# anibali/dsnt-pose2d

Hardware: AMD Instinct MI355X
Metric: images/sec (train step, 256x256, 16 joints) (higher is better)
Workload: dtype f32; 1 GPU; hg2 + DSNT + JS reg, 256x256 -> 64x64x16, batch 32 per GPU, RMSprop lr 2.5e-4, train step fwd+loss+bwd+optim; global_batch=32, parallelism=dp1, launches_fwd=212

## Files before the change

dsnt-pose2d_amd/csrc/api.cpp:

```cpp
#include "common.h"
#include "stage.h"
#include <string.h>

static thread_local char g_err[512] = "";

int dsnt_set_error(int code, const char* fmt, ...) {
    va_list ap;
    va_start(ap, fmt);
    vsnprintf(g_err, sizeof(g_err), fmt, ap);
    va_end(ap);
    return code;
}

int dsnt_device_id(void) {
    int d = 0;
    if (hipGetDevice(&d) != hipSuccess || d < 0) d = 0;
    return d < DSNT_MAX_DEVICES ? d : DSNT_MAX_DEVICES - 1;
}

int dsnt_device_cus(void) {
    static std::atomic<int> cus[DSNT_MAX_DEVICES];
    const int d = dsnt_device_id();
    int c = cus[d].load(std::memory_order_acquire);
    if (!c) {
        hipDeviceProp_t prop;
        int dev = 0;
        c = (hipGetDevice(&dev) == hipSuccess && hipGetDeviceProperties(&prop, dev) == hipSuccess && prop.multiProcessorCount > 0)
                ? prop.multiProcessorCount : 256;
        cus[d].store(c, std::memory_order_release);
    }
    return c;
}

extern "C" int dsnt_version(void) { return 121; }
extern "C" const char* dsnt_last_error(void) { return g_err; }

#include <vector>
#include <new>

struct dsnt_list {
    struct Entry {
        int kind;
        int lane, src, dst;
        mutable hipEvent_t ev;
        std::function<void(hipStream_t)> fn;
        int st_code = 0, gx = 0, gy = 0, nt = 0;
        std::vector<unsigned char> params;
        int fused = 0;
        unsigned* st_sync = nullptr;
// ... 202 lines not shown
```

dsnt-pose2d_amd/csrc/head.hip:

```cpp
#include "common.h"
#include "flipmerge.h"
#include <math.h>

#define HB 256

template <int VEC, bool CACHED, typename SRC = const float*>
struct Row {
    float v[16];
    SRC src;
    int hw;
    __device__ __forceinline__ void load(SRC row, int n) {
        src = row; hw = n;
        if (CACHED) {
            const int tid = threadIdx.x;
            if (VEC == 4) {
#pragma unroll
                for (int k = 0; k < 4; ++k) {
                    const int i = (k * HB + tid) * 4;
                    float4 t = make_float4(0.f, 0.f, 0.f, 0.f);
                    if (i < hw) t = row_load4(row, i);
                    v[4 * k] = t.x; v[4 * k + 1] = t.y; v[4 * k + 2] = t.z; v[4 * k + 3] = t.w;
                }
            } else {
#pragma unroll
// ... 612 lines not shown
        float x, y; g.xy(i, x, y);
        float v = ax * x + ay * y;
        if (kind >= 0 && gr != 0.f) v += gr * reg_grad(p, x, y, c, tx, ty, k, sigma, kind);
        return v;
    };
    float s[1] = {0.f};
    row.each([&](int i, float p) { s[0] = fmaf(p, dLdp(i, p), s[0]); });
    block_sum<1>(s, red);
    float* out = g_logits + r * hw;
    row.each([&](int i, float p) { out[i] = p * (dLdp(i, p) - s[0]); });
}

#define HEAD_SEP_MAX 512
#define LN2 0.69314718055994530942f

template <int VEC>
__global__ __launch_bounds__(HB) void head_loss_grad_kernel(const float* __restrict__ hm, const float* __restrict__ coords,
                                                            const float* __restrict__ target, const float* __restrict__ mask,
                                                            const float* __restrict__ denom_p, float* __restrict__ dist_out,
                                                            float* __restrict__ reg_out, float* __restrict__ g0, int h, int w,
                                                            float sigma, float k, int kind, float reg_coeff) {
    __shared__ float red[16];
    __shared__ __attribute__((aligned(16))) float exy[HEAD_SEP_MAX];
    __shared__ __attribute__((aligned(16))) float pos[HEAD_SEP_MAX];
    const size_t r = blockIdx.x;
    const int hw = h * w;
    const float tx = target[2 * r], ty = target[2 * r + 1];
    const float cx = coords[2 * r], cy = coords[2 * r + 1];
    const float mk = mask ? mask[r] : 1.f;
    const float den = denom_p[1];
    Row<VEC, true> row;
    row.load(hm + r * hw, hw);
    const Grid2 g(h, w);
    const float dxm = cx - tx, dym = cy - ty;
    const float d = sqrtf(dxm * dxm + dym * dym);
    const float wm = mk / den;
    const float f = wm / (2.f * d);
    const float ax = f * (2.f * dxm), ay = f * (2.f * dym);
    const float gr = kind >= 0 ? wm * reg_coeff : 0.f;
    float gv[16];
    float acc[2] = {0.f, 0.f};
    const bool tab = w + h <= HEAD_SEP_MAX;
    if (tab) {
        for (int i = threadIdx.x; i < w + h; i += HB)
            pos[i] = i < w ? (2.f * i - g.offx) / (float)w : (2.f * (i - w) - g.offy) / (float)h;
    }
    if (kind == 0 && tab) {
// ... 87 lines not shown
                    const float4 xv = *reinterpret_cast<const float4*>(pos + cc);
                    one(4 * kk, row.v[4 * kk], xv.x, y); one(4 * kk + 1, row.v[4 * kk + 1], xv.y, y);
                    one(4 * kk + 2, row.v[4 * kk + 2], xv.z, y); one(4 * kk + 3, row.v[4 * kk + 3], xv.w, y);
                }
            }
        } else {
            row.each_slot([&](int slot, int i, float p) {
                float x, y; g.xy(i, x, y);
                one(slot, p, x, y);
            });
        }
        float s1[1] = {acc[1]};
        block_sum<1>(s1, red);
        acc[0] = val; acc[1] = s1[0];
    }
    float* out = g0 + r * hw;
    if (VEC == 4) {
#pragma unroll
        for (int kk = 0; kk < 4; ++kk) {
            const int i = (kk * HB + threadIdx.x) * 4;
            if (i < hw)
                *reinterpret_cast<float4*>(out + i) = make_float4(row.v[4 * kk] * (gv[4 * kk] - acc[1]), row.v[4 * kk + 1] * (gv[4 * kk + 1] - acc[1]),
                                                                  row.v[4 * kk + 2] * (gv[4 * kk + 2] - acc[1]), row.v[4 * kk + 3] * (gv[4 * kk + 3] - acc[1]));
        }
    } else {
        row.each_slot([&](int slot, int i, float p) { out[i] = p * (gv[slot] - acc[1]); });
    }
    if (threadIdx.x == 0) {
        dist_out[r] = d;
        if (reg_out) reg_out[r] = acc[0];
    }
}

__global__ __launch_bounds__(HB) void mask_denom_kernel(const float* __restrict__ m, float* __restrict__ out2, long n) {
    __shared__ float red[16];
    float s[1] = {0.f};
    for (long i = threadIdx.x; i < n; i += HB) s[0] += m ? m[i] : 1.f;
    block_sum<1>(s, red);
    if (threadIdx.x == 0) { out2[0] = s[0]; out2[1] = fmaxf(s[0], 1.f); }
}

__global__ __launch_bounds__(HB) void head_loss_reduce_kernel(const float* __restrict__ dist, const float* __restrict__ reg,
                                                              const float* __restrict__ m, const float* __restrict__ denom2,
                                                              float reg_coeff, float* __restrict__ loss, float* __restrict__ e2,
                                                              long n) {
    __shared__ float red[16];
// ... 11 lines not shown
        loss[0] = reg ? a + reg_coeff * (s[1] / den) : a;
    }
}

__global__ void scale_by_scalar_kernel(float* __restrict__ x, const float* __restrict__ s, long n4, long n) {
    const float a = s[0];
    if (a == 1.f) return;
    const long t0 = (long)blockIdx.x * blockDim.x + threadIdx.x, step = (long)gridDim.x * blockDim.x;
    float4* x4 = reinterpret_cast<float4*>(x);
    for (long i = t0; i < n4; i += step) {
        float4 v = x4[i];
        v.x *= a; v.y *= a; v.z *= a; v.w *= a;
        x4[i] = v;
    }
    for (long i = 4 * n4 + t0; i < n; i += step) x[i] *= a;
}

#define ROW_DISPATCH(KERNEL, rows, hw, ptr_ok, ...)                                                   \
    do {                                                                                               \
        const bool vec_ = ((hw) % 4 == 0) && (ptr_ok);                                                 \
        const bool cached_ = (hw) <= 4096;                                                             \
        hipStream_t st_ = (hipStream_t)stream;                                                         \
        if (vec_ && cached_) DSNT_LAUNCH((KERNEL<4, true>), dim3(rows), dim3(HB), 0, st_, __VA_ARGS__);   \
        else if (cached_) DSNT_LAUNCH((KERNEL<1, true>), dim3(rows), dim3(HB), 0, st_, __VA_ARGS__);      \
        else DSNT_LAUNCH((KERNEL<1, false>), dim3(rows), dim3(HB), 0, st_, __VA_ARGS__);                  \
    } while (0)

static int check_rows(const char* who, int64_t rows, int h, int w) {
    DSNT_REQUIRE(rows > 0 && rows < (1LL << 31), DSNT_ERR_SHAPE, "%s: rows=%lld out of range", who, (long long)rows);
    DSNT_REQUIRE(h > 0 && w > 0 && (long)h * w < (1L << 24), DSNT_ERR_SHAPE, "%s: bad map size %dx%d", who, h, w);
// ... 301 lines not shown
    DSNT_REQUIRE(dist && denom2 && loss && e2 && rows > 0, DSNT_ERR_ARG, "dsnt_head_loss_reduce: bad argument");
    DSNT_LAUNCH(head_loss_reduce_kernel, dim3(1), dim3(HB), 0, (hipStream_t)stream, dist, reg_row, mask, denom2, reg_coeff,
                       loss, e2, (long)rows);
    DSNT_CHECK_LAUNCH("dsnt_head_loss_reduce");
}

extern "C" int dsnt_scale_by_scalar(float* x, const float* s, int64_t n, void* stream) {
    DSNT_REQUIRE(x && s && n > 0, DSNT_ERR_ARG, "dsnt_scale_by_scalar: null pointer or n <= 0");
    const long n4 = dsnt_aligned16(x) ? (long)(n / 4) : 0;
    long gsz = ((n4 ? n4 : (long)n) + 255) / 256;
    if (gsz > 4096) gsz = 4096;
    DSNT_LAUNCH(scale_by_scalar_kernel, dim3((unsigned)gsz), dim3(256), 0, (hipStream_t)stream, x, s, n4, (long)n);
    DSNT_CHECK_LAUNCH("dsnt_scale_by_scalar");
}

__global__ __launch_bounds__(256) void fc2_fwd_kernel(const float* __restrict__ hm, const float* __restrict__ w,
                                                      const float* __restrict__ b, float* __restrict__ out, int hw) {
    __shared__ float red[2][4];
    const float* row = hm + (size_t)blockIdx.x * hw;
    float a0 = 0.f, a1 = 0.f;
    for (int i = threadIdx.x; i < hw; i += 256) {
        const float v = row[i];
        a0 = fmaf(v, w[i], a0);
        a1 = fmaf(v, w[hw + i], a1);
    }
    for (int o = 32; o >= 1; o >>= 1) { a0 += __shfl_xor(a0, o); a1 += __shfl_xor(a1, o); }
    if ((threadIdx.x & 63) == 0) { red[0][threadIdx.x >> 6] = a0; red[1][threadIdx.x >> 6] = a1; }
    __syncthreads();
    if (threadIdx.x < 2) {
        const float s = red[threadIdx.x][0] + red[threadIdx.x][1] + red[threadIdx.x][2] + red[threadIdx.x][3];
// ... 43 lines not shown
```

dsnt-pose2d_amd/dsnt/_lib.py:

```python
import ctypes as C
import os

import torch

_HERE = os.path.dirname(os.path.abspath(__file__))
LIB_PATH = os.environ.get('DSNT_HIP_LIB') or os.path.join(os.path.dirname(_HERE), 'csrc', 'libdsnt_hip.so')

P = C.c_void_p
I = C.c_int
L = C.c_int64
F = C.c_float
D = C.c_double


class ConvGeom(C.Structure):
    _fields_ = [(n, C.c_int) for n in
                ('N', 'H', 'W', 'Cin', 'Ho', 'Wo', 'Cout', 'R', 'S', 'stride', 'pad', 'dil')]


GP = C.POINTER(ConvGeom)


class BnBwdEpilogue(C.Structure):
    _fields_ = [('x', C.c_void_p), ('scale', C.c_void_p), ('shift', C.c_void_p), ('mean', C.c_void_p),
# ... 46 lines not shown
    'dsnt_reg_bwd_mu': [P, P, P, P, L, I, I, F, I, P],
    'dsnt_euclid_fwd': [P, P, P, L, I, P],
    'dsnt_euclid_bwd': [P, P, P, P, P, L, I, P],
    'dsnt_masked_avg_fwd': [P, P, P, L, P],
    'dsnt_masked_avg_bwd': [P, P, P, P, L, P],
    'dsnt_head_fwd': [P, P, P, L, I, I, P],
    'dsnt_flip_merge_head': [P, L, I, I, I, P, I, I, F, F, P, P, P, P, P, P],
    'dsnt_flip_merge_head_stats': [P, L, I, I, I, P, I, I, F, F, P, P, P, P, P, P, P, P, P],
    'dsnt_heatmap_stats': [P, L, I, I, P, P, P],
    'dsnt_head_loss_rows': [P, P, P, P, P, L, I, I, F, I, P],
    'dsnt_head_bwd': [P, P, P, P, P, P, P, L, I, I, F, I, P],
    'dsnt_head_loss_grad': [P, P, P, P, P, P, P, P, L, I, I, F, I, F, P],
    'dsnt_mask_denom': [P, P, L, P],
    'dsnt_head_loss_reduce': [P, P, P, P, F, P, P, L, P],
    'dsnt_scale_by_scalar': [P, P, L, P],
    'dsnt_conv_fwd': [P, P, P, P, P, P, I, P, P, P, GP, P],
    'dsnt_conv_fwd_ex': [P, P, P, P, P, P, I, P, P, P, GP, BP, TP, P],
    'dsnt_conv_fwd_bf16x6_ex': [P, P, L, P, P, P, P, I, P, P, P, GP, BP, TP, P],
    'dsnt_conv_pack_dgrad': [P, P, I, I, I, I, P],
    'dsnt_conv_pack_dgrad_all': [P, I, P, P, P, L, P],
    'dsnt_conv_fwd_bf16x6': [P, P, L, P, P, P, P, I, P, P, P, GP, P],
    'dsnt_split_bf16x3': [P, P, L, P],
    'dsnt_conv_fwd_f16x3_ex': [P, P, L, P, P, P, P, P, P, I, P, P, P, GP, BP, TP, P],
    'dsnt_conv_fwd_f16x3_stream': [P, P, L, P, P, P, P, P, P, I, P, P, P, GP, BP, TP, P],
    'dsnt_amax': [P, L, P, P],
    'dsnt_split_f16x2': [P, P, L, L, P, P],
    'dsnt_f16_prep_weights': [P, I, I, P],
    'dsnt_f16_prep_bn_bounds': [P, I, P],
    'dsnt_conv_wgrad': [P, P, P, I, P, P, P, P, I, GP, P],
    'dsnt_conv_wgrad_bf16x6': [P, P, P, I, P, P, P, P, I, GP, P],
# ... 166 lines not shown
```

dsnt-pose2d_amd/dsnt/engine.py:

```python
import ctypes as C
import os

import torch

from . import _lib
from ._lib import ConvGeom, BnBwdEpilogue, BnTail, BnPrologue, BnBwdApply

BN_EPS = 1e-5
BN_MOMENTUM = 0.1


class Act:
    __slots__ = ('buf', 'N', 'H', 'W', 'C', '_grad', 'stats', 'name', 'grad_amax', 'amax_tail', 'fold_ok',
                 'pending_apply', 'uses', 'gives_away', 'is_branch', 'grad_shared', 'pending_add', 'base', 'base_amax')

    def __init__(self, buf, name=''):
        self.buf = buf
        self.N, self.H, self.W, self.C = buf.shape
        self._grad = None
        self.base, self.base_amax = None, None
        self.stats = None
        self.amax_tail = None
        self.grad_amax = None
        self.fold_ok = False
# ... 1237 lines not shown

    def to_planar(self, x, C_logical, name='', out=None, gin=None):
        out = self.empty(x.N, C_logical, x.H, x.W) if out is None else out
        x.uses += 1
        if gin is None:
            gin = self.empty(x.N, C_logical, x.H, x.W) if self.record else None
        self.f('dsnt_nhwc_to_nchw', x.buf, out, x.N, C_logical, x.H * x.W, x.C)
        if self.record:
            def backward():
                assert x.grad is None, 'planar output must be the first gradient writer'
                buf, _ = self.grad_target(x)
                self.b('dsnt_nchw_to_nhwc', gin, buf, x.N, C_logical, x.H * x.W, x.C)
            self.on_backward(backward)
        return out, gin

    def from_planar(self, src_nchw, Cpad, name=''):
        N, Cc, H, W = src_nchw.shape
        a = self.act(N, H, W, Cpad, name)
        e = self.f('dsnt_nchw_to_nhwc', src_nchw, a.buf, N, Cc, H * W, Cpad)
        self._planar_src[id(a)] = (src_nchw, e)
        return a

    def stem_s2d(self, x, p, name='stem'):
        got = self._planar_src.get(id(x))
        if (got is None or not self.use_f16x3 or not self.stem_s2d_on or p.R != 7 or p.S != 7 or p.stride != 2 or p.pad != 3
                or p.dil != 1 or x.C != 4 or x.H % 2 or x.W % 2 or x.N * (x.H // 2) * (x.W // 2) < self.bf16x6_min_rows):
            return None
        src, entry = got
        self.fwd.remove(entry)
        xs = self.act(x.N, x.H // 2 + 1, x.W // 2 + 1, 16, 'input_s2d')
# ... 15 lines not shown
```

dsnt-pose2d_amd/dsnt/hourglass.py:

```python
import os

import torch
import torch.nn as nn
from torch.autograd import Function

from . import _lib
from .engine import Tape, ConvParams, BnParams

EXPANSION = 2


def _ceil4(n):
    return (n + 3) // 4 * 4


class Arena:

    def __init__(self, module, device):
        self.device = device
        self.publish_scale = 1.0
        slots, off = [], 0
        skip = tuple(getattr(module, 'tape_exclude', ()))
        named = [(n, p) for n, p in module.named_parameters() if not (skip and n.startswith(skip))]
        bucket_of = getattr(module, 'param_bucket', lambda name: 0)
# ... 93 lines not shown
                fresh = self.fresh[o:o + n] * a
                if p.dim() == 4:
                    O, I, R, S = p.shape
                    fresh = fresh.view(O, R, S, _ceil4(I)).permute(0, 3, 1, 2)[:, :I]
                else:
                    fresh = fresh.view(p.shape)
                if p.grad is None:
                    self.gviews[name].copy_(fresh)
                    p.grad = self.gviews[name]
                else:
                    p.grad.add_(fresh)


class Program:

    def __init__(self, root, arena, in_shape, training, input_grad, record=None):
        self.training = training
        self.record = record = training if record is None else bool(record)
        self.token = 0
        self.in_flight = False
        self.owner = None
        dev = arena.device
        tape = Tape(dev, training, record)
        tape.want_input_grad = bool(input_grad and record)
        tape.param_arena = arena.params
        self.tape = tape
        names = {id(m): n for n, m in root.named_modules()}

        def key(m, leaf):
            prefix = names[id(m)]
            return (prefix + '.' if prefix else '') + leaf
# ... 26 lines not shown
        N, Cc, H, W = in_shape
        prep_pos = len(tape.fwd)
        if tape.use_bf16x6:
            tape.f('dsnt_split_bf16x3', arena.params, arena.planes, arena.numel)
        prep_head = tuple(tape.fwd[prep_pos:])
        self.in_nchw = tape.empty(N, Cc, H, W)
        x = tape.from_planar(self.in_nchw, _ceil4(Cc), 'input')
        self.in_act = x
        outs = root.trace(tape, x, P)
        single = not isinstance(outs, (list, tuple))
        self.single = single
        outs = [outs] if single else list(outs)
        self.out_channels = root.out_channels
        self.outs, self.gins = [], []
        self.out_slab = self.gin_slab = None
        if not single and len(outs) > 1 and len({(o.N, o.H, o.W) for o in outs}) == 1 and os.environ.get('DSNT_STACKED_OUTPUTS', '1') != '0':
            o = outs[0]
            self.out_slab = tape.empty(len(outs), o.N, self.out_channels, o.H, o.W)
            self.gin_slab = tape.empty(len(outs), o.N, self.out_channels, o.H, o.W) if record else None
        for i, o in enumerate(outs):
            t, g = tape.to_planar(o, self.out_channels, out=None if self.out_slab is None else self.out_slab[i],
                                  gin=None if self.gin_slab is None else self.gin_slab[i])
            self.outs.append(t)
            self.gins.append(g)
        self.input_grad = input_grad and record
        if record:
            tape.finish()
        tape.emit_f16_prep(prep_pos, prep_head)
        if record:
            if self.input_grad:
                self.gx = tape.empty(N, Cc, H, W)
                if x.grad is None:
                    raise RuntimeError('input gradient requested but nothing produced it')
                tape.b('dsnt_nhwc_to_nchw', x.grad, self.gx, N, Cc, H * W, x.C)
        self.n_fwd = sum(1 for e in tape.fwd if e[0] is not None)
        self.n_bwd = sum(1 for e in tape.bwd if e[0] is not None)


class StackedOutputs(list):

    def __init__(self, stacked):
        super().__init__(stacked.unbind(0))
        self.stacked = stacked


class _Run(Function):
    @staticmethod
    def forward(ctx, runner, prog, x, *params):
        import weakref
        prog.in_nchw.copy_(x)
        prog.token += 1
        prog.tape.run(prog.tape.fwd, probe=runner.probe)
        ctx.runner, ctx.prog, ctx.token, ctx.nparams = runner, prog, prog.token, len(params)
        prog.in_flight = True
        token = prog.owner = prog.token

        def release(p=prog, t=token):
            if p.owner == t:
                p.in_flight, p.owner = False, None
        weakref.finalize(ctx, release)
        if prog.out_slab is not None:
            return (prog.out_slab.clone(),)
        return tuple(o.clone() for o in prog.outs)

    @staticmethod
    def backward(ctx, *gouts):
        prog, runner = ctx.prog, ctx.runner
        if not prog.record:
            raise RuntimeError('dsnt: this forward was traced without a backward list')
        if prog.token != ctx.token:
            if prog.owner == ctx.token:
                prog.in_flight, prog.owner = False, None
            raise RuntimeError('dsnt: the saved activations of this forward were overwritten by a '
                               'later forward of the same shape; run backward before forwarding again')
        if prog.gin_slab is not None:
            if gouts[0] is None:
                prog.gin_slab.zero_()
            else:
                prog.gin_slab.copy_(gouts[0])
        else:
            for g, gin in zip(gouts, prog.gins):
                if g is None:
                    gin.zero_()
                else:
                    gin.copy_(g)
        prog.tape.run(prog.tape.bwd, runner.bucket_hook, probe=runner.probe)
        if runner.before_publish is not None:
            runner.before_publish()
        runner.arena.publish_grads(runner.params)
        prog.in_flight = False
# ... 2 lines not shown
        return (None, None, gx) + (None,) * ctx.nparams


class Runner:
    MAX_IN_FLIGHT = 4

    def __init__(self, root):
        self.root = root
        self.arena = None
        self.programs = {}
        self.params = []
        self._bns = None
        self.probe = None
        self.bucket_hook = None
        self.before_publish = None

    def ensure(self, device):
        if self.arena is None or not self.arena.valid() or self.arena.device != device:
            self.arena = Arena(self.root, device)
            self.programs = {}
            self.params = [p for _, p, _, _ in self.arena.slots]

    def _bn_signature(self):
        if self._bns is None:
            self._bns = [m for m in self.root.modules() if isinstance(m, nn.BatchNorm2d)]
        return tuple((m.momentum, m.eps) for m in self._bns)

    def __call__(self, x):
        if not x.is_cuda:
            raise RuntimeError('dsnt: input is on %s; the backbone runs on the HIP device only '
                               '(no CPU fallback) — move the model and input with .cuda()' % x.device)
        if x.dtype != torch.float32:
            raise RuntimeError('dsnt: expected a float32 input, got %s' % x.dtype)
        self.ensure(x.device)
        training = self.root.training
        grad_mode = torch.is_grad_enabled()
        record = grad_mode and (training or x.requires_grad or any(p.requires_grad for p in self.params))
        key = (tuple(x.shape), training, bool(x.requires_grad), self._bn_signature()) + (('eval+backward',) if (record and not training) else ())
        prog = self.programs.get(key)
        if prog is not None and prog.in_flight and (record or training):
            k = 1
            while (key, k) in self.programs and self.programs[(key, k)].in_flight:
                k += 1
            if k >= self.MAX_IN_FLIGHT:
                raise RuntimeError('dsnt: %d forward passes of this shape are waiting for their backward; run backward (or drop the '
                                   'outputs) before forwarding again' % k)
            key = (key, k)
            prog = self.programs.get(key)
        if prog is None:
            if x.requires_grad and not self.root.supports_input_grad:
                raise NotImplementedError('dsnt: gradient with respect to the input image is not '
                                          'on the hot path (stride-2 stem data-gradient)')
            prog = Program(self.root, self.arena, tuple(x.shape), training, bool(x.requires_grad), record=record or training)
            self.programs[key] = prog
        if record:
            outs = _Run.apply(self, prog, x, *self.params)
        else:
            with torch.no_grad():
                prog.in_nchw.copy_(x)
                prog.token += 1
                prog.tape.run(prog.tape.fwd, probe=self.probe)
                outs = (prog.out_slab.clone(),) if prog.out_slab is not None else tuple(o.clone() for o in prog.outs)
        if prog.out_slab is not None:
            return StackedOutputs(outs[0])
        return outs[0] if prog.single else list(outs)


class TapeModule(nn.Module):
    supports_input_grad = True

    def _runner(self):
        r = self.__dict__.get('_tape_runner')
        if r is None:
            r = Runner(self)
            self.__dict__['_tape_runner'] = r
        return r

# ... 180 lines not shown
```

dsnt-pose2d_amd/dsnt/model.py:

```python
import inspect
import re

import torch
from torch import nn

from . import nn as dnn
from . import util as dutil
from . import hourglass
from . import resnet
from .data import ImageSpecs


class HumanPoseModel(nn.Module):

    def _hm_preact(self, x, preact):
        return dnn.hm_preact(x, preact)

    def _calculate_reg_loss(self, target_var, mask_var, reg, hm_var, hm_sigma):
        sigma = 2.0 * hm_sigma / hm_var.size(-1)
        if reg == 'var':
            return dnn.variance_reg_loss(hm_var, target_var, sigma, mask_var)
        if reg == 'kl':
            return dnn.kl_reg_loss(hm_var, target_var, sigma, mask_var)
        if reg == 'js':
# ... 34 lines not shown

    @property
    def image_specs(self):
        return ImageSpecs(size=256, subtract_mean=True, divide_stddev=False)

    @property
    def heatmaps(self):
        return self.heatmaps_array[0]

    def forward_part1(self, x):
        return self.hg(x)

    def forward_part2(self, hg_outs):
        out = []
        self._fused = {}
        if self.output_strat == 'gauss':
            self.heatmaps_array = hg_outs
            return hg_outs
        self._fused_all = None
        stacked = getattr(hg_outs, 'stacked', None)
        if self.output_strat == 'dsnt' and self.preact == 'softmax' and stacked is not None and stacked.dim() == 5:
            S = stacked.size(0)
            x4 = stacked.reshape(-1, stacked.size(-3), stacked.size(-2), stacked.size(-1))
            hm, coords = dnn.head_forward(x4)
            out = list(coords.view(S, -1, coords.size(-2), 2).unbind(0))
            self.heatmaps_array = list(hm.view(stacked.shape).unbind(0))
            self._fused_all = (x4, hm, coords, out)
            return out
        if self.output_strat == 'dsnt':
            self.heatmaps_array = []
            for x in hg_outs:
                if self.preact == 'softmax':
                    x4 = x.reshape(-1, x.size(-3), x.size(-2), x.size(-1))
                    hm, coords = dnn.head_forward(x4)
# ... 2 lines not shown
                    hm = self._hm_preact(x, self.preact)
                    coords = dnn.dsnt(hm)
                self.heatmaps_array.append(hm)
                out.append(coords)
            return out
        if self.output_strat == 'fc':
            self.heatmaps_array = []
            for x in hg_outs:
                hm = self._hm_preact(x, self.preact)
                self.heatmaps_array.append(hm)
                out.append(dnn.fc_coords(hm, self.out_fc.weight, self.out_fc.bias).view(-1, self.n_chans, 2))
            return out
        raise Exception('invalid configuration')

    def forward(self, *inputs):
        return self.forward_part2(self.forward_part1(inputs[0]))

    def forward_loss(self, out_vars, target_var, mask_var):
        if self.output_strat == 'dsnt' or self.output_strat == 'fc':
            total_loss = 0
            denom2 = None
            fa = getattr(self, '_fused_all', None)
            if fa is not None and len(out_vars) == len(fa[3]) and all(a is b for a, b in zip(out_vars, fa[3])):
                x4, hm, coords, out = fa
                S, rows = len(out), coords.numel() // 2 // len(out)
                sigma = 2.0 * self.hm_sigma / hm.size(-1)
                m_ = None if mask_var is None else mask_var.to(torch.float32).expand(out[0].shape[:-1])
                denom2 = dnn.mask_denominator(m_, rows, hm.device)
                t_all = target_var.to(torch.float32).expand_as(out[0]).unsqueeze(0).expand(S, *out[0].shape).reshape(coords.shape)
                m_all = None if m_ is None else m_.unsqueeze(0).expand(S, *m_.shape).reshape(coords.shape[:-1])
                return dnn.head_loss(x4, hm.detach(), coords.detach(), t_all, m_all, self.reg, sigma, self.reg_coeff, denom2)
            if fa is not None:
                x4, hm, coords, out = fa
                S = len(out)
                x5, hm5 = x4.view(S, -1, *x4.shape[1:]), hm.view(S, -1, *hm.shape[1:])
                for s_, o in enumerate(out):
# ... 161 lines not shown
```

dsnt-pose2d_amd/dsnt/nn.py:

```python
import math

import numpy as np
import torch
from torch.autograd import Function

from . import _lib
from ._lib import ptr, f32, call

PREACT_MODES = {'softmax': 0, 'thresholded_softmax': 1, 'abs': 2, 'relu': 3, 'sigmoid': 4}
REG_KINDS = {'js': 0, 'kl': 1, 'mse': 2, 'var': 3}


def _rows(t, trailing):
    n = 1
    for s in t.shape[:t.dim() - trailing]:
        n *= s
    return n


def generate_xy(inp):
    h, w = inp.shape[-2], inp.shape[-1]
    lead = [1] * (inp.dim() - 2)
    xs = torch.linspace(-(w - 1) / w, (w - 1) / w, w, device=inp.device).view(*lead, 1, w)
    ys = torch.linspace(-(h - 1) / h, (h - 1) / h, h, device=inp.device).view(*lead, h, 1)
# ... 345 lines not shown
        rows = _rows(hm, 2)
        g1 = f32(g).contiguous().view(1)
        if ctx.g0 is not None:
            g_logits, ctx.g0 = ctx.g0, None
            call('dsnt_scale_by_scalar', ptr(g_logits), ptr(g1), g_logits.numel())
            return g_logits, None, None, None, None, None, None, None, None
        g_dist = torch.empty(rows, device=hm.device, dtype=hm.dtype)
        call('dsnt_masked_avg_bwd', ptr(g1), ptr(m), ptr(e2), ptr(g_dist), rows)
        g_reg = (g_dist * ctx.reg_coeff) if ctx.kind >= 0 else None
        g_logits = torch.empty_like(hm)
        call('dsnt_head_bwd', ptr(hm), ptr(coords), ptr(t), ptr(dist), ptr(g_dist), ptr(g_reg),
             ptr(g_logits), rows, h, w, ctx.sigma, ctx.kind)
        return g_logits, None, None, None, None, None, None, None, None


def mask_denominator(mask, rows, device):
    m = None if mask is None else f32(mask).contiguous()
    out = torch.empty(2, device=device, dtype=torch.float32)
    call('dsnt_mask_denom', ptr(m), ptr(out), rows)
    return out


def head_loss(logits, hm, coords, target, mask, reg, sigma, reg_coeff, denom2=None):
    kind = REG_KINDS.get(reg, -1)
    return _HeadLoss.apply(logits, hm, coords, target, mask, kind, float(sigma), float(reg_coeff), denom2)
```

include/dsnt_hip.h:

```cpp
#ifndef DSNT_HIP_H
#define DSNT_HIP_H

#include <stdint.h>

#ifdef __cplusplus
extern "C" {
#endif

typedef enum {
    DSNT_OK = 0,
    DSNT_ERR_SHAPE = 1,
    DSNT_ERR_ALIGN = 2,
    DSNT_ERR_ARG = 3,
    DSNT_ERR_HIP = 4
} dsnt_status;

typedef struct {
    float* amax;
    float* amax_bn; const float* amax_scale; const float* amax_shift; int amax_relu, reserved;
} dsnt_out_bounds;

typedef struct dsnt_bn_prologue {
    const float* partial; int tiles, C;
    int64_t M;
// ... 51 lines not shown
int dsnt_heatmap_stats(const float* hm, int64_t rows, int h, int w, float* stats, int* peak_index, void* stream);
int dsnt_flip_merge_head_stats(const float* logits, int64_t B, int J, int h, int w, const int* perm, int strategy,
                               int preact, float threshold, float eps, const double* transform_m,
                               const double* transform_b, float* hm, float* coords, double* img, float* stats,
                               int* peak_index, double* cov_image, void* stream);
int dsnt_head_loss_rows(const float* hm, const float* coords, const float* target,
                        float* dist, float* reg_row, int64_t rows, int h, int w, float sigma,
                        int reg_kind, void* stream);
int dsnt_mask_denom(const float* mask, float* denom2, int64_t n, void* stream);
int dsnt_head_loss_grad(const float* hm, const float* coords, const float* target, const float* mask,
                        const float* denom2, float* dist, float* reg_row, float* g_logits, int64_t rows, int h, int w,
                        float sigma, int reg_kind, float reg_coeff, void* stream);
int dsnt_head_loss_reduce(const float* dist, const float* reg_row, const float* mask, const float* denom2,
                          float reg_coeff, float* loss, float* e2, int64_t rows, void* stream);
int dsnt_scale_by_scalar(float* x, const float* s, int64_t n, void* stream);
int dsnt_head_bwd(const float* hm, const float* coords, const float* target, const float* dist,
                  const float* g_dist, const float* g_reg, float* g_logits, int64_t rows,
                  int h, int w, float sigma, int reg_kind, void* stream);

typedef struct {
    int N, H, W, Cin;
    int Ho, Wo, Cout;
    int R, S;
    int stride, pad, dil;
} dsnt_conv_geom;

int dsnt_conv_fwd(const float* x, const float* w, const float* bias, float* y,
                  const float* in_scale, const float* in_shift, int in_relu,
                  const float* res1, const float* res2, float* stats_partial,
                  const dsnt_conv_geom* g, void* stream);
// ... 284 lines not shown
```

Baseline: 2878 images/sec.

## Read and write the DSNT head directly in NHWC hourglass layout

Adds NHWC-aware head kernels. They read logits straight from the hourglass's padded NHWC activation buffers and write loss gradients directly into an NHWC gradient slab that is exposed to the tape. This skips the planar output slab clone, the NHWC to NCHW conversions and the separate mask-denominator launch, and folds the mask scaling into the gradient store. The cost is strided per-channel global accesses in the head kernels, which are less coalesced than planar rows. It also brings a more complex autograd contract, which raises an error when gradients arrive through both paths.

```diff
diff --git a/dsnt-pose2d_amd/csrc/api.cpp b/dsnt-pose2d_amd/csrc/api.cpp
--- a/dsnt-pose2d_amd/csrc/api.cpp
+++ b/dsnt-pose2d_amd/csrc/api.cpp
@@ -32,7 +32,7 @@
     return c;
 }
 
-extern "C" int dsnt_version(void) { return 121; }
+extern "C" int dsnt_version(void) { return 122; }
 extern "C" const char* dsnt_last_error(void) { return g_err; }
 
 #include <vector>
diff --git a/dsnt-pose2d_amd/csrc/head.hip b/dsnt-pose2d_amd/csrc/head.hip
--- a/dsnt-pose2d_amd/csrc/head.hip
+++ b/dsnt-pose2d_amd/csrc/head.hip
@@ -650,23 +650,24 @@
 #define HEAD_SEP_MAX 512
 #define LN2 0.69314718055994530942f
 
-template <int VEC>
-__global__ __launch_bounds__(HB) void head_loss_grad_kernel(const float* __restrict__ hm, const float* __restrict__ coords,
-                                                            const float* __restrict__ target, const float* __restrict__ mask,
-                                                            const float* __restrict__ denom_p, float* __restrict__ dist_out,
-                                                            float* __restrict__ reg_out, float* __restrict__ g0, int h, int w,
-                                                            float sigma, float k, int kind, float reg_coeff) {
-    __shared__ float red[16];
-    __shared__ __attribute__((aligned(16))) float exy[HEAD_SEP_MAX];
-    __shared__ __attribute__((aligned(16))) float pos[HEAD_SEP_MAX];
-    const size_t r = blockIdx.x;
+struct HeadLossLds {
+    float red[16];
+    __attribute__((aligned(16))) float exy[HEAD_SEP_MAX];
+    __attribute__((aligned(16))) float pos[HEAD_SEP_MAX];
+};
+
+template <int VEC, typename SINK>
+__device__ __forceinline__ void head_loss_grad_row(const float* __restrict__ hm_row, float tx, float ty, float cx, float cy,
+                                                   float mk, float den, float* __restrict__ dist_out,
+                                                   float* __restrict__ reg_out, const SINK& sink, int h, int w, float sigma,
+                                                   float k, int kind, float reg_coeff, HeadLossLds& lds,
+                                                   float row_scale = 1.f) {
+    float* red = lds.red;
+    float* exy = lds.exy;
+    float* pos = lds.pos;
     const int hw = h * w;
-    const float tx = target[2 * r], ty = target[2 * r + 1];
-    const float cx = coords[2 * r], cy = coords[2 * r + 1];
-    const float mk = mask ? mask[r] : 1.f;
-    const float den = denom_p[1];
     Row<VEC, true> row;
-    row.load(hm + r * hw, hw);
+    row.load(hm_row, hw);
     const Grid2 g(h, w);
     const float dxm = cx - tx, dym = cy - ty;
     const float d = sqrtf(dxm * dxm + dym * dym);
@@ -784,22 +785,44 @@
         block_sum<1>(s1, red);
         acc[0] = val; acc[1] = s1[0];
     }
-    float* out = g0 + r * hw;
     if (VEC == 4) {
 #pragma unroll
         for (int kk = 0; kk < 4; ++kk) {
             const int i = (kk * HB + threadIdx.x) * 4;
             if (i < hw)
-                *reinterpret_cast<float4*>(out + i) = make_float4(row.v[4 * kk] * (gv[4 * kk] - acc[1]), row.v[4 * kk + 1] * (gv[4 * kk + 1] - acc[1]),
-                                                                  row.v[4 * kk + 2] * (gv[4 * kk + 2] - acc[1]), row.v[4 * kk + 3] * (gv[4 * kk + 3] - acc[1]));
+                sink.store4(i, make_float4(row.v[4 * kk] * (gv[4 * kk] - acc[1]), row.v[4 * kk + 1] * (gv[4 * kk + 1] - acc[1]),
+                                           row.v[4 * kk + 2] * (gv[4 * kk + 2] - acc[1]), row.v[4 * kk + 3] * (gv[4 * kk + 3] - acc[1])));
         }
     } else {
-        row.each_slot([&](int slot, int i, float p) { out[i] = p * (gv[slot] - acc[1]); });
+        row.each_slot([&](int slot, int i, float p) { sink.store1(i, p * (gv[slot] - acc[1])); });
     }
     if (threadIdx.x == 0) {
-        dist_out[r] = d;
-        if (reg_out) reg_out[r] = acc[0];
-    }
+        *dist_out = d * row_scale;
+        if (reg_out) *reg_out = acc[0] * row_scale;
+    }
+}
+
+struct PlanarSink {
+    float* out;
+    __device__ __forceinline__ void store4(int i, float4 v) const { *reinterpret_cast<float4*>(out + i) = v; }
+    __device__ __forceinline__ void store1(int i, float v) const { out[i] = v; }
+};
+
+template <int VEC>
+__global__ __launch_bounds__(HB) void head_loss_grad_kernel(const float* __restrict__ hm, const float* __restrict__ coords,
+                                                            const float* __restrict__ target, const float* __restrict__ mask,
+                                                            const float* __restrict__ denom_p, float* __restrict__ dist_out,
+                                                            float* __restrict__ reg_out, float* __restrict__ g0, int h, int w,
+                                                            float sigma, float k, int kind, float reg_coeff) {
+    __shared__ HeadLossLds lds;
+    const size_t r = blockIdx.x;
+    const int hw = h * w;
+    const float tx = target[2 * r], ty = target[2 * r + 1];
+    const float cx = coords[2 * r], cy = coords[2 * r + 1];
+    const float mk = mask ? mask[r] : 1.f;
+    const float den = denom_p[1];
+    head_loss_grad_row<VEC>(hm + r * hw, tx, ty, cx, cy, mk, den, dist_out + r, reg_out ? reg_out + r : nullptr,
+                            PlanarSink{g0 + r * hw}, h, w, sigma, k, kind, reg_coeff, lds);
 }
 
 __global__ __launch_bounds__(HB) void mask_denom_kernel(const float* __restrict__ m, float* __restrict__ out2, long n) {
@@ -841,6 +864,79 @@
         x4[i] = v;
     }
     for (long i = 4 * n4 + t0; i < n; i += step) x[i] *= a;
+}
+
+struct NhwcSrc {
+    const float* p;
+    int stride;
+    __device__ __forceinline__ float operator[](int i) const { return p[(size_t)i * stride]; }
+};
+__device__ __forceinline__ float4 row_load4(const NhwcSrc& s, int i) { return make_float4(s[i], s[i + 1], s[i + 2], s[i + 3]); }
+
+__device__ __forceinline__ bool nhwc_row(int J, int images, int& img, int& j) {
+    const int b = blockIdx.x;
+    img = (b & 7) + 8 * (b / (8 * J));
+    j = (b >> 3) % J;
+    return img < images;
+}
+
+template <int VEC>
+__global__ __launch_bounds__(HB) void head_fwd_nhwc_kernel(const float* const* __restrict__ logits, float* __restrict__ hm,
+                                                            float* __restrict__ coords, int S, int N, int J, int h, int w,
+                                                            int Cpad) {
+    __shared__ float red[16];
+    int img, j;
+    if (!nhwc_row(J, S * N, img, j)) return;
+    const int s = img / N, n = img - s * N, hw = h * w;
+    const size_t r = (size_t)img * J + j;
+    Row<VEC, true, NhwcSrc> row;
+    row.load(NhwcSrc{logits[s] + (size_t)n * hw * Cpad + j, Cpad}, hw);
+    float c[2];
+    head_fwd_row<VEC, true, true>(row, hm + r * hw, h, w, red, c);
+    if (threadIdx.x == 0) { coords[2 * r] = c[0]; coords[2 * r + 1] = c[1]; }
+}
+
+struct NhwcSink {
+    float* out;
+    int stride, pad;
+    float scale;
+    __device__ __forceinline__ void store1(int i, float v) const {
+        float* o = out + (size_t)i * stride;
+        o[0] = v * scale;
+        for (int c = 1; c <= pad; ++c) o[c] = 0.f;
+    }
+    __device__ __forceinline__ void store4(int i, float4 v) const {
+        store1(i, v.x); store1(i + 1, v.y); store1(i + 2, v.z); store1(i + 3, v.w);
+    }
+};
+
+template <int VEC>
+__global__ __launch_bounds__(HB) void head_loss_grad_nhwc_kernel(const float* __restrict__ hm, const float* __restrict__ coords,
+                                                                  const float* __restrict__ target, const float* __restrict__ mask,
+                                                                  const float* __restrict__ upstream, float* __restrict__ denom2,
+                                                                  float* __restrict__ dist_out, float* __restrict__ reg_out,
+                                                                  float* const* __restrict__ grads,
+                                                                  int S, int N, int J, int h, int w, int Cpad, float sigma,
+                                                                  float k, int kind, float reg_coeff) {
+    __shared__ HeadLossLds lds;
+    int img, j;
+    if (!nhwc_row(J, S * N, img, j)) return;
+    const int s = img / N, n = img - s * N, hw = h * w;
+    const size_t r = (size_t)img * J + j;
+    const int tj = n * J + j;
+    const float tx = target[2 * tj], ty = target[2 * tj + 1];
+    const float cx = coords[2 * r], cy = coords[2 * r + 1];
+    const float mk = mask ? mask[tj] : 1.f;
+    const float up = upstream ? upstream[0] : 1.f;
+    float sm[1] = {0.f};
+    for (int i = threadIdx.x; i < N * J; i += HB) sm[0] += mask ? mask[i] : 1.f;
+    block_sum<1>(sm, lds.red);
+    const float den = fmaxf(sm[0], 1.f);
+    if (denom2 && blockIdx.x == 0 && threadIdx.x == 0) { denom2[0] = sm[0]; denom2[1] = den; }
+    __syncthreads();
+    const NhwcSink sink{grads[s] + (size_t)n * hw * Cpad + j, Cpad, j == J - 1 ? Cpad - J : 0, up};
+    head_loss_grad_row<VEC>(hm + r * hw, tx, ty, cx, cy, mk, den, dist_out + r, reg_out ? reg_out + r : nullptr, sink, h, w,
+                            sigma, k, kind, reg_coeff, lds, mk);
 }
 
 #define ROW_DISPATCH(KERNEL, rows, hw, ptr_ok, ...)                                                   \
@@ -1172,6 +1268,47 @@
     DSNT_CHECK_LAUNCH("dsnt_scale_by_scalar");
 }
 
+static int check_nhwc(const char* who, int S, int N, int J, int h, int w, int Cpad) {
+    DSNT_REQUIRE(S > 0 && N > 0 && J > 0 && Cpad >= J && Cpad % 4 == 0, DSNT_ERR_SHAPE,
+                 "%s: S=%d N=%d J=%d Cpad=%d (Cpad >= J, a multiple of 4)", who, S, N, J, Cpad);
+    DSNT_REQUIRE(h > 0 && w > 0 && (long)h * w <= 4096, DSNT_ERR_SHAPE, "%s: heat-maps of up to 4096 pixels (got %dx%d); "
+                 "larger ones take the planar kernels", who, h, w);
+    DSNT_REQUIRE((long)S * N * J < (1L << 27), DSNT_ERR_SHAPE, "%s: %ld rows", who, (long)S * N * J);
+    return DSNT_OK;
+}
+
+static inline unsigned nhwc_grid(int S, int N, int J) { return (unsigned)(((long)S * N + 7) / 8 * 8 * J); }
+
+extern "C" int dsnt_head_fwd_nhwc(const float* const* logits, float* hm, float* coords, int S, int N, int J, int h, int w,
+                                  int Cpad, void* stream) {
+    DSNT_REQUIRE(logits && hm && coords, DSNT_ERR_ARG, "dsnt_head_fwd_nhwc: null tensor");
+    if (int e = check_nhwc("dsnt_head_fwd_nhwc", S, N, J, h, w, Cpad)) return e;
+    hipStream_t st = (hipStream_t)stream;
+    if ((h * w) % 4 == 0 && dsnt_aligned16(hm))
+        DSNT_LAUNCH(head_fwd_nhwc_kernel<4>, dim3(nhwc_grid(S, N, J)), dim3(HB), 0, st, logits, hm, coords, S, N, J, h, w, Cpad);
+    else
+        DSNT_LAUNCH(head_fwd_nhwc_kernel<1>, dim3(nhwc_grid(S, N, J)), dim3(HB), 0, st, logits, hm, coords, S, N, J, h, w, Cpad);
+    DSNT_CHECK_LAUNCH("dsnt_head_fwd_nhwc");
+}
+
+extern "C" int dsnt_head_loss_grad_nhwc(const float* hm, const float* coords, const float* target, const float* mask,
+                                        const float* upstream, float* denom2, float* dist, float* reg_row,
+                                        float* const* g_logits, int S, int N, int J, int h, int w, int Cpad, float sigma,
+                                        int reg_kind, float reg_coeff, void* stream) {
+    DSNT_REQUIRE(hm && coords && target && dist && g_logits && (reg_kind < 0 || reg_row), DSNT_ERR_ARG,
+                 "dsnt_head_loss_grad_nhwc: null tensor");
+    DSNT_REQUIRE(reg_kind >= -1 && reg_kind <= 3, DSNT_ERR_ARG, "dsnt_head_loss_grad_nhwc: unknown regulariser %d", reg_kind);
+    if (int e = check_nhwc("dsnt_head_loss_grad_nhwc", S, N, J, h, w, Cpad)) return e;
+    hipStream_t st = (hipStream_t)stream;
+    if ((h * w) % 4 == 0 && dsnt_aligned16(hm))
+        DSNT_LAUNCH(head_loss_grad_nhwc_kernel<4>, dim3(nhwc_grid(S, N, J)), dim3(HB), 0, st, hm, coords, target, mask, upstream,
+                    denom2, dist, reg_row, g_logits, S, N, J, h, w, Cpad, sigma, gauss_k(sigma), reg_kind, reg_coeff);
+    else
+        DSNT_LAUNCH(head_loss_grad_nhwc_kernel<1>, dim3(nhwc_grid(S, N, J)), dim3(HB), 0, st, hm, coords, target, mask, upstream,
+                    denom2, dist, reg_row, g_logits, S, N, J, h, w, Cpad, sigma, gauss_k(sigma), reg_kind, reg_coeff);
+    DSNT_CHECK_LAUNCH("dsnt_head_loss_grad_nhwc");
+}
+
 __global__ __launch_bounds__(256) void fc2_fwd_kernel(const float* __restrict__ hm, const float* __restrict__ w,
                                                       const float* __restrict__ b, float* __restrict__ out, int hw) {
     __shared__ float red[2][4];
diff --git a/dsnt-pose2d_amd/dsnt/_lib.py b/dsnt-pose2d_amd/dsnt/_lib.py
--- a/dsnt-pose2d_amd/dsnt/_lib.py
+++ b/dsnt-pose2d_amd/dsnt/_lib.py
@@ -84,6 +84,8 @@
     'dsnt_mask_denom': [P, P, L, P],
     'dsnt_head_loss_reduce': [P, P, P, P, F, P, P, L, P],
     'dsnt_scale_by_scalar': [P, P, L, P],
+    'dsnt_head_fwd_nhwc': [P, P, P, I, I, I, I, I, I, P],
+    'dsnt_head_loss_grad_nhwc': [P, P, P, P, P, P, P, P, P, I, I, I, I, I, I, F, I, F, P],
     'dsnt_conv_fwd': [P, P, P, P, P, P, I, P, P, P, GP, P],
     'dsnt_conv_fwd_ex': [P, P, P, P, P, P, I, P, P, P, GP, BP, TP, P],
     'dsnt_conv_fwd_bf16x6_ex': [P, P, L, P, P, P, P, I, P, P, P, GP, BP, TP, P],
diff --git a/dsnt-pose2d_amd/dsnt/engine.py b/dsnt-pose2d_amd/dsnt/engine.py
--- a/dsnt-pose2d_amd/dsnt/engine.py
+++ b/dsnt-pose2d_amd/dsnt/engine.py
@@ -1275,6 +1275,15 @@
             self.on_backward(backward)
         return out, gin
 
+    def expose_nhwc(self, x, grad):
+        assert tuple(grad.shape) == (x.N, x.H, x.W, x.C)
+        x.uses += 1
+        if self.record:
+            def backward():
+                assert x.grad is None, 'an exposed output must be the first gradient writer'
+                x.grad = grad
+            self.on_backward(backward)
+
     def from_planar(self, src_nchw, Cpad, name=''):
         N, Cc, H, W = src_nchw.shape
         a = self.act(N, H, W, Cpad, name)
diff --git a/dsnt-pose2d_amd/dsnt/hourglass.py b/dsnt-pose2d_amd/dsnt/hourglass.py
--- a/dsnt-pose2d_amd/dsnt/hourglass.py
+++ b/dsnt-pose2d_amd/dsnt/hourglass.py
@@ -131,7 +131,7 @@
 
 class Program:
 
-    def __init__(self, root, arena, in_shape, training, input_grad, record=None):
+    def __init__(self, root, arena, in_shape, training, input_grad, record=None, head_nhwc=False):
         self.training = training
         self.record = record = training if record is None else bool(record)
         self.token = 0
@@ -188,6 +188,11 @@
         self.out_channels = root.out_channels
         self.outs, self.gins = [], []
         self.out_slab = self.gin_slab = None
+        self.head = None
+        stackable = not single and len(outs) > 1 and len({(o.N, o.H, o.W, o.C) for o in outs}) == 1 and os.environ.get('DSNT_STACKED_OUTPUTS', '1') != '0'
+        if head_nhwc and stackable and record and training and not input_grad and outs[0].H * outs[0].W <= 4096:
+            self.head = NhwcHead(tape, outs, self.out_channels)
+            outs = []
         if not single and len(outs) > 1 and len({(o.N, o.H, o.W) for o in outs}) == 1 and os.environ.get('DSNT_STACKED_OUTPUTS', '1') != '0':
             o = outs[0]
             self.out_slab = tape.empty(len(outs), o.N, self.out_channels, o.H, o.W)
@@ -211,6 +216,26 @@
         self.n_bwd = sum(1 for e in tape.bwd if e[0] is not None)
 
 
+class NhwcHead:
+
+    def __init__(self, tape, outs, J):
+        o = outs[0]
+        self.S, self.N, self.J, self.H, self.W, self.Cpad = len(outs), o.N, J, o.H, o.W, o.C
+        self.grad_slab = tape.empty(self.S, o.N, o.H, o.W, o.C)
+        for i, a in enumerate(outs):
+            tape.expose_nhwc(a, self.grad_slab[i])
+        self.logits = [a.buf for a in outs]
+        table = lambda ts: torch.tensor([t.data_ptr() for t in ts], dtype=torch.int64).to(tape.device)
+        self.logits_table, self.grads_table = table(self.logits), table(list(self.grad_slab.unbind(0)))
+
+
+class NhwcLogits(list):
+
+    def __init__(self, head, token):
+        super().__init__()
+        self.head, self.token, self.state = head, token, {}
+
+
 class StackedOutputs(list):
 
     def __init__(self, stacked):
@@ -233,6 +258,8 @@
             if p.owner == t:
                 p.in_flight, p.owner = False, None
         weakref.finalize(ctx, release)
+        if prog.head is not None:
+            return (torch.empty(1, device=x.device),)
         if prog.out_slab is not None:
             return (prog.out_slab.clone(),)
         return tuple(o.clone() for o in prog.outs)
@@ -247,7 +274,9 @@
                 prog.in_flight, prog.owner = False, None
             raise RuntimeError('dsnt: the saved activations of this forward were overwritten by a '
                                'later forward of the same shape; run backward before forwarding again')
-        if prog.gin_slab is not None:
+        if prog.head is not None:
+            pass
+        elif prog.gin_slab is not None:
             if gouts[0] is None:
                 prog.gin_slab.zero_()
             else:
@@ -280,6 +309,7 @@
         self.probe = None
         self.bucket_hook = None
         self.before_publish = None
+        self.head_nhwc = False
 
     def ensure(self, device):
         if self.arena is None or not self.arena.valid() or self.arena.device != device:
@@ -303,6 +333,9 @@
         grad_mode = torch.is_grad_enabled()
         record = grad_mode and (training or x.requires_grad or any(p.requires_grad for p in self.params))
         key = (tuple(x.shape), training, bool(x.requires_grad), self._bn_signature()) + (('eval+backward',) if (record and not training) else ())
+        head_nhwc = bool(self.head_nhwc and record and training and not x.requires_grad)
+        if head_nhwc:
+            key = key + ('head_nhwc',)
         prog = self.programs.get(key)
         if prog is not None and prog.in_flight and (record or training):
             k = 1
@@ -317,7 +350,8 @@
             if x.requires_grad and not self.root.supports_input_grad:
                 raise NotImplementedError('dsnt: gradient with respect to the input image is not '
                                           'on the hot path (stride-2 stem data-gradient)')
-            prog = Program(self.root, self.arena, tuple(x.shape), training, bool(x.requires_grad), record=record or training)
+            prog = Program(self.root, self.arena, tuple(x.shape), training, bool(x.requires_grad), record=record or training,
+                           head_nhwc=head_nhwc)
             self.programs[key] = prog
         if record:
             outs = _Run.apply(self, prog, x, *self.params)
@@ -327,6 +361,8 @@
                 prog.token += 1
                 prog.tape.run(prog.tape.fwd, probe=self.probe)
                 outs = (prog.out_slab.clone(),) if prog.out_slab is not None else tuple(o.clone() for o in prog.outs)
+        if prog.head is not None:
+            return NhwcLogits(prog.head, outs[0])
         if prog.out_slab is not None:
             return StackedOutputs(outs[0])
         return outs[0] if prog.single else list(outs)
diff --git a/dsnt-pose2d_amd/dsnt/model.py b/dsnt-pose2d_amd/dsnt/model.py
--- a/dsnt-pose2d_amd/dsnt/model.py
+++ b/dsnt-pose2d_amd/dsnt/model.py
@@ -1,4 +1,5 @@
 import inspect
+import os
 import re
 
 import torch
@@ -72,10 +73,17 @@
     def forward_part2(self, hg_outs):
         out = []
         self._fused = {}
+        self._fused_nhwc = None
         if self.output_strat == 'gauss':
             self.heatmaps_array = hg_outs
             return hg_outs
         self._fused_all = None
+        if isinstance(hg_outs, hourglass.NhwcLogits):
+            hm, coords = dnn.head_forward_nhwc(hg_outs)
+            out = list(coords.unbind(0))
+            self.heatmaps_array = list(hm.unbind(0))
+            self._fused_nhwc = (hg_outs, hm, coords, out)
+            return out
         stacked = getattr(hg_outs, 'stacked', None)
         if self.output_strat == 'dsnt' and self.preact == 'softmax' and stacked is not None and stacked.dim() == 5:
             S = stacked.size(0)
@@ -108,12 +116,28 @@
         raise Exception('invalid configuration')
 
     def forward(self, *inputs):
-        return self.forward_part2(self.forward_part1(inputs[0]))
+        runner = None
+        if (self.output_strat == 'dsnt' and self.preact == 'softmax' and isinstance(self.hg, hourglass.TapeModule)
+                and 'headnhwc' not in os.environ.get('DSNT_OFF', '').replace('+', ',').split(',')):
+            runner = self.hg._runner()
+            runner.head_nhwc = True
+        try:
+            hg_outs = self.forward_part1(inputs[0])
+        finally:
+            if runner is not None:
+                runner.head_nhwc = False
+        return self.forward_part2(hg_outs)
 
     def forward_loss(self, out_vars, target_var, mask_var):
         if self.output_strat == 'dsnt' or self.output_strat == 'fc':
             total_loss = 0
             denom2 = None
+            fn = getattr(self, '_fused_nhwc', None)
+            if fn is not None and len(out_vars) == len(fn[3]) and all(a is b for a, b in zip(out_vars, fn[3])):
+                nh, hm, coords, out = fn
+                sigma = 2.0 * self.hm_sigma / hm.size(-1)
+                m_ = None if mask_var is None else mask_var.to(torch.float32)
+                return dnn.head_loss_nhwc(nh, hm.detach(), coords.detach(), target_var.to(torch.float32), m_, self.reg, sigma, self.reg_coeff)
             fa = getattr(self, '_fused_all', None)
             if fa is not None and len(out_vars) == len(fa[3]) and all(a is b for a, b in zip(out_vars, fa[3])):
                 x4, hm, coords, out = fa
diff --git a/dsnt-pose2d_amd/dsnt/nn.py b/dsnt-pose2d_amd/dsnt/nn.py
--- a/dsnt-pose2d_amd/dsnt/nn.py
+++ b/dsnt-pose2d_amd/dsnt/nn.py
@@ -383,6 +383,96 @@
         return g_logits, None, None, None, None, None, None, None, None
 
 
+_MIXED = ('dsnt: the gradient of this forward reached the logits both through forward_loss and through the outputs themselves; '
+          'the NHWC head writes one of them — set DSNT_OFF=headnhwc for such a loss')
+
+
+class _HeadForwardNhwc(Function):
+
+    @staticmethod
+    def forward(ctx, token, nh):
+        h = nh.head
+        hm = torch.empty(h.S, h.N, h.J, h.H, h.W, device=token.device, dtype=torch.float32)
+        coords = torch.empty(h.S, h.N, h.J, 2, device=token.device, dtype=torch.float32)
+        call('dsnt_head_fwd_nhwc', ptr(h.logits_table), ptr(hm), ptr(coords), h.S, h.N, h.J, h.H, h.W, h.Cpad)
+        ctx.nh = nh
+        ctx.set_materialize_grads(False)
+        ctx.save_for_backward(hm)
+        return hm, coords
+
+    @staticmethod
+    def backward(ctx, g_hm, g_coords):
+        (hm,) = ctx.saved_tensors
+        nh, h = ctx.nh, ctx.nh.head
+        if nh.state.get('loss'):
+            raise RuntimeError(_MIXED)
+        nh.state['outputs'] = True
+        rows = _rows(hm, 2)
+        g = None
+        if g_coords is not None:
+            g = torch.empty_like(hm)
+            call('dsnt_expect_bwd', ptr(f32(g_coords).contiguous()), ptr(g), rows, h.H, h.W)
+        if g_hm is not None:
+            g = g_hm.contiguous() if g is None else g + g_hm
+        if g is None:
+            g = torch.zeros_like(hm)
+        gx = torch.empty_like(hm)
+        call('dsnt_preact_bwd', None, ptr(hm), ptr(g), ptr(gx), rows, h.H * h.W, 0, 0.0, 0.0)
+        for s in range(h.S):
+            call('dsnt_nchw_to_nhwc', ptr(gx[s]), ptr(h.grad_slab[s]), h.N, h.J, h.H * h.W, h.Cpad)
+        return hm.new_empty(1), None
+
+
+def head_forward_nhwc(nh):
+    return _HeadForwardNhwc.apply(nh.token, nh)
+
+
+class _HeadLossNhwc(Function):
+
+    @staticmethod
+    def forward(ctx, token, nh, hm, coords, target, mask, kind, sigma, reg_coeff):
+        h = nh.head
+        rows = h.S * h.N * h.J
+        t = f32(target).expand(h.N, h.J, 2).contiguous()
+        m = None if mask is None else f32(mask).expand(h.N, h.J).contiguous()
+        dist = torch.empty(rows, device=hm.device, dtype=hm.dtype)
+        reg = torch.empty(rows, device=hm.device, dtype=hm.dtype) if kind >= 0 else None
+        denom2 = torch.empty(2, device=hm.device, dtype=hm.dtype)
+        call('dsnt_head_loss_grad_nhwc', ptr(hm), ptr(coords), ptr(t), ptr(m), None, ptr(denom2), ptr(dist), ptr(reg),
+             ptr(h.grads_table), h.S, h.N, h.J, h.H, h.W, h.Cpad, sigma, kind, reg_coeff)
+        out = torch.empty(3, device=hm.device, dtype=hm.dtype)
+        e2 = out[1:]
+        call('dsnt_head_loss_reduce', ptr(dist), ptr(reg), None, ptr(denom2), reg_coeff, ptr(out), ptr(e2), rows)
+        ctx.save_for_backward(hm, coords, t, m)
+        ctx.nh, ctx.kind, ctx.sigma, ctx.reg_coeff = nh, kind, sigma, reg_coeff
+        ctx.tag = nh.state['grad_of'] = object()
+        return out[0]
+
+    @staticmethod
+    def backward(ctx, g):
+        hm, coords, t, m = ctx.saved_tensors
+        nh, h = ctx.nh, ctx.nh.head
+        if nh.state.get('outputs'):
+            raise RuntimeError(_MIXED)
+        nh.state['loss'] = True
+        g1 = f32(g).contiguous().view(1)
+        if nh.state.get('grad_of') is ctx.tag:
+            nh.state['grad_of'] = None
+            call('dsnt_scale_by_scalar', ptr(h.grad_slab), ptr(g1), h.grad_slab.numel())
+        else:
+            rows = h.S * h.N * h.J
+            dist = torch.empty(rows, device=hm.device, dtype=hm.dtype)
+            reg = torch.empty(rows, device=hm.device, dtype=hm.dtype) if ctx.kind >= 0 else None
+            call('dsnt_head_loss_grad_nhwc', ptr(hm), ptr(coords), ptr(t), ptr(m), ptr(g1), None, ptr(dist), ptr(reg),
+                 ptr(h.grads_table), h.S, h.N, h.J, h.H, h.W, h.Cpad, ctx.sigma, ctx.kind, ctx.reg_coeff)
+        return hm.new_empty(1), None, None, None, None, None, None, None, None
+
+
+def head_loss_nhwc(nh, hm, coords, target, mask, reg, sigma, reg_coeff):
+    kind = REG_KINDS.get(reg, -1)
+    return _HeadLossNhwc.apply(nh.token, nh, hm, coords, target, mask, kind, float(sigma), float(reg_coeff))
+
+
 def mask_denominator(mask, rows, device):
     m = None if mask is None else f32(mask).contiguous()
     out = torch.empty(2, device=device, dtype=torch.float32)
diff --git a/include/dsnt_hip.h b/include/dsnt_hip.h
--- a/include/dsnt_hip.h
+++ b/include/dsnt_hip.h
@@ -89,6 +89,11 @@
 int dsnt_head_loss_reduce(const float* dist, const float* reg_row, const float* mask, const float* denom2,
                           float reg_coeff, float* loss, float* e2, int64_t rows, void* stream);
 int dsnt_scale_by_scalar(float* x, const float* s, int64_t n, void* stream);
+int dsnt_head_fwd_nhwc(const float* const* logits, float* hm, float* coords, int S, int N, int J, int h, int w, int Cpad,
+                       void* stream);
+int dsnt_head_loss_grad_nhwc(const float* hm, const float* coords, const float* target, const float* mask,
+                             const float* upstream, float* denom2, float* dist, float* reg_row, float* const* g_logits, int S,
+                             int N, int J, int h, int w, int Cpad, float sigma, int reg_kind, float reg_coeff, void* stream);
 int dsnt_head_bwd(const float* hm, const float* coords, const float* target, const float* dist,
                   const float* g_dist, const float* g_reg, float* g_logits, int64_t rows,
                   int h, int w, float sigma, int reg_kind, void* stream);
```

Result: no change. 2889 images/sec (median of 6 runs) (+0.4%).
